# RKWin93/E2E-MAPPO-for-MT-FJSP

Measured on AMD Instinct MI355X. Metric: env-steps/sec (batched J6M6E2), higher is better.
Workload: dtype f64 (environment) / f32 (encoder: f32 storage and accumulation; 128x128 products on the 16-bit matrix cores from split f32 operands, f32-accurate: DESIGN.md §4)

## Files before the change

### __graft_entry__.py

```python
#!/usr/bin/env python3
import os
import sys

ROOT = os.path.dirname(os.path.abspath(__file__))
if ROOT not in sys.path:
    sys.path.insert(0, ROOT)


def build() -> None:
    from importlib import import_module
    import mtfjsp_amd
    _build = import_module("e2e-mappo-for-mt-fjsp_amd._build")
    lib = _build.build(force=True, verbose=True)
    capi = import_module("e2e-mappo-for-mt-fjsp_amd.capi")
    capi.lib()
    print("variant:", _build.build_variant("funcs", ["-DMTFJSP_BODY_FUNCS=3"]))
    from oracle import env_oracle
    print("oracle:", env_oracle.build(force=True))
    print("built", lib)


def smoke() -> None:
    import numpy as np
    import torch
    from importlib import import_module
    import mtfjsp_amd
    assert torch.cuda.is_available(), "smoke() needs cuda:0"
    batch_env = import_module("e2e-mappo-for-mt-fjsp_amd.batch_env")
    inst = import_module("e2e-mappo-for-mt-fjsp_amd.instances")
    from oracle.env_oracle import OracleBatch
    J, M, E, B = 6, 6, 2, 8
    T = J * M
    t, p, tt, edge = inst.generate_instances(B, J, M, E, seed=0)
    import random
    random.seed(0)
    w3 = inst.random_weights(B)
    env = batch_env.DeviceBatchEnv(J, M, E, B, obs_dtype="f64")
    env.load_instances(t, p, tt, edge=edge)
    env.scaler_init()
    env.reset(w3)
    orc = OracleBatch(t, p, tt, edge)
    orc.scaler_init()
    orc.reset(w3)
    a = torch.zeros(B, dtype=torch.int32, device=env.device); m = torch.zeros_like(a); j = torch.zeros_like(a)
    for s in range(T):
        env.random_actions(7, s, a, m, j)
        env.step(a, m)
        info, raw, _ = orc.step(a.cpu().numpy(), m.cpu().numpy())
        cand, mask = orc.job_mask_update(j.cpu().numpy())
        o = orc.observe()
        assert np.array_equal(env.info.cpu().numpy(), info), f"step {s}: rewards differ"
        assert np.array_equal(env.tasks_fea.cpu().numpy(), o["tfea"]), f"step {s}: tasks_fea differ"
        assert np.array_equal(env.dense_adj().cpu().numpy(), o["adj"]), f"step {s}: adj differ"
        assert np.array_equal(env.m_fea2.cpu().numpy(), o["mfea2"])
        assert np.array_equal(env.candidate.cpu().numpy(), cand) and np.array_equal(env.job_mask.cpu().numpy(), mask)
    assert bool(env.info[:, 1].all())
    _smoke_encoder()
    print("smoke OK: HIP env == oracle on", B, "instances x", T, "steps")


def _smoke_encoder() -> None:
    try:
        from importlib import import_module
        enc = import_module("e2e-mappo-for-mt-fjsp_amd.encoder")
    except ImportError:
        return
    if hasattr(enc, "smoke"):
        enc.smoke()


if __name__ == "__main__":
    cmd = sys.argv[1] if len(sys.argv) > 1 else "build"
    {"build": build, "smoke": smoke}[cmd]()
```

### e2e-mappo-for-mt-fjsp_amd/csrc/mtfjsp_gin_resident.h

```cpp
#pragma once
#include <type_traits>
#include <utility>

#ifndef GR_ABL
#define GR_ABL 0
#endif
#define GR_NT 18
#ifndef GR_NRES
#define GR_NRES 16
#endif
#ifndef GR_VRES
#define GR_VRES 1
#endif
#define GR_ROWS (32 * GR_NT)
#define GR_RING 6
#define GR_NBAR 6
#ifndef GR_GRP
#define GR_GRP 2
#endif
#ifndef GR_LOOK
#define GR_LOOK 2
#endif
#define GR_ROWB 272
#define GR_PLANE (32 * GR_ROWB)
#define GR_TILE (2 * GR_PLANE)
#define GR_MAXCAND 384
#define GR_MAXWARM 10
#define GR_MAXT 65
#define GR_MINT 16
#define GR_MAXIPC 64

#ifndef GR_MIX
#define GR_MIX 2
#endif
#ifndef GR_SETTLE
#define GR_SETTLE 1
#endif
#ifndef GR_FOLD_DPP
#define GR_FOLD_DPP 1
#endif
#ifndef GR_STAT_ASM
#define GR_STAT_ASM 0
#endif
#ifndef GR_PK
#define GR_PK 1
#endif
typedef float f32x16 __attribute__((ext_vector_type(16)));
typedef _Float16 gr_h8 __attribute__((ext_vector_type(8)));
typedef _Float16 gr_h2 __attribute__((ext_vector_type(2)));

struct GinResArgs {
    int B, T, J, ipc;
    const void *tfea; int feat_f64;
    const int *ell_col; const float *ell_val;
    const void *Wx32[6];
    float wsinv[6];
    const float *gamma[6], *beta[6];
    unsigned long long *stats;
    unsigned long long *stats_next;
    int wexp[6];
    int ffrac[6];
    unsigned long long *bar;
    unsigned long long epoch;
    unsigned *fail;
    unsigned *range_flag;
    const int *candidate;
    float *pooled;
    float *cand_feat;
    float *h_nodes;
    float *zspill;
    double inv_rows;
    int barrier_only;
    unsigned expect_extra;
    unsigned long long *stamps;
    const void *warm[GR_MAXWARM];
    unsigned warm_lines[GR_MAXWARM];
    int nwarm;
};
#define GR_STATS_PART (6 * 8 * HD * 2)
#define GR_STATS_SET GR_STATS_PART
#ifdef GR_STAMP
#define GR_STAMP_AT(i) do { if (tid == 0 && A.stamps) { A.stamps[(size_t)blockIdx.x * 64 + (i)] = __builtin_amdgcn_s_memrealtime(); \
                                                         if ((i) <= 30) A.stamps[(size_t)blockIdx.x * 64 + 33 + (i)] = __builtin_amdgcn_s_memtime(); } } while (0)
#else
#define GR_STAMP_AT(i) do { } while (0)
#endif

#define GR_OFF_PLANES 0
#define GR_OFF_RING (2 * GR_TILE)
#define GR_RING_BYTES ((2 * GR_LOOK - 2) * GR_TILE > GR_RING * 32 * HD * 4 ? (2 * GR_LOOK - 2) * GR_TILE : GR_RING * 32 * HD * 4)
#define GR_OFF_ELLC (GR_OFF_RING + GR_RING_BYTES)
#define GR_OFF_ELLV0 (GR_OFF_ELLC + GR_ROWS * 4)
#define GR_OFF_ELLV1 (GR_OFF_ELLV0 + GR_ROWS * 4)
#define GR_OFF_BN (GR_OFF_ELLV1 + GR_ROWS * 4)
#define GR_OFF_CAND (GR_OFF_BN + 2 * HD * 4)
#define GR_OFF_ZERO (GR_OFF_CAND + GR_ROWS * 4)
#define GR_OFF_FLAG (GR_OFF_ZERO + 2 * HD * 4)
#define GR_OFF_CNT (GR_OFF_FLAG + 64)
#define GR_LDS_BYTES (GR_OFF_CNT + 5 * (GR_NT / GR_GRP) * 4 + 12)
static size_t gin_res_lds_bytes() { return (size_t)GR_LDS_BYTES; }
static_assert(GR_LDS_BYTES <= 160 * 1024, "resident GIN kernel: LDS budget");

#if GR_PK == 1
__device__ __forceinline__ f32x2 gr_fma2(f32x2 a, f32x2 b, f32x2 c) { return __builtin_elementwise_fma(a, b, c); }
__device__ __forceinline__ f32x2 gr_add2(f32x2 a, f32x2 b) { return a + b; }
__device__ __forceinline__ f32x2 gr_sub2(f32x2 a, f32x2 b) { return a - b; }
__device__ __forceinline__ f32x2 gr_mul2(f32x2 a, f32x2 b) { return a * b; }
#else
#if GR_PK == 2
__device__ __forceinline__ float gr_pin(float x) { return x; }
#else
__device__ __forceinline__ float gr_pin(float x) { asm("" : "+v"(x)); return x; }
#endif
__device__ __forceinline__ f32x2 gr_fma2(f32x2 a, f32x2 b, f32x2 c) { return f32x2{gr_pin(__builtin_fmaf(a[0], b[0], c[0])), gr_pin(__builtin_fmaf(a[1], b[1], c[1]))}; }
__device__ __forceinline__ f32x2 gr_add2(f32x2 a, f32x2 b) { return f32x2{gr_pin(a[0] + b[0]), gr_pin(a[1] + b[1])}; }
__device__ __forceinline__ f32x2 gr_sub2(f32x2 a, f32x2 b) { return f32x2{gr_pin(a[0] - b[0]), gr_pin(a[1] - b[1])}; }
__device__ __forceinline__ f32x2 gr_mul2(f32x2 a, f32x2 b) { return f32x2{gr_pin(a[0] * b[0]), gr_pin(a[1] * b[1])}; }
#endif
__device__ __forceinline__ f32x2 gr_rem2(f32x2 v, gr_h2 p)
// ... 128 lines not shown
#pragma unroll
        for (int k = 0; k < NER; k++) {
            const int r = tid + 256 * k, rc = r < nrows ? r : nrows - 1;
            ecc[k] = *reinterpret_cast<const int2 *>(A.ell_col + (grow0 + rc) * 2);
            evv[k] = *reinterpret_cast<const float2 *>(A.ell_val + (grow0 + rc) * 2);
        }
#pragma unroll
        for (int k = 0; k < NF4; k++) reinterpret_cast<f32x4 *>(s_feat)[tid + 256 * k] = fpre[k];
        if (A.feat_f64) {
            const double *src = reinterpret_cast<const double *>(A.tfea) + grow0 * 12;
            const int n12 = nrows * 12;
            __syncthreads();
#pragma unroll 1
            for (int i0 = 0; i0 < n12; i0 += 256 * 9) {
                double d[9];
#pragma unroll
                for (int k = 0; k < 9; k++) { const int i = i0 + tid + 256 * k; d[k] = src[i < n12 ? i : n12 - 1]; }
#pragma unroll
                for (int k = 0; k < 9; k++) { const int i = i0 + tid + 256 * k; if (i < n12) s_feat[i] = (float)d[k]; }
            }
        }
#pragma unroll
        for (int k = 0; k < NER; k++) {
            const int r = tid + 256 * k;
            if (r < GR_ROWS) {
                unsigned cp = 0xffffffffu; float v0 = 0.f, v1 = 0.f;
                if (r < nrows) {
                    const int2 cc = ecc[k];
                    const float2 vv = evv[k];
                    const int base = (r / T) * T;
                    const unsigned r0 = cc.x >= 0 ? (unsigned)(base + cc.x) : 0xffffu, r1 = cc.y >= 0 ? (unsigned)(base + cc.y) : 0xffffu;
                    cp = r0 | (r1 << 16); v0 = cc.x >= 0 ? vv.x : 0.f; v1 = cc.y >= 0 ? vv.y : 0.f;
                }
                s_ellc[r] = cp; s_ellv0[r] = v0; s_ellv1[r] = v1; s_rowcand[r] = -1;
            }
        }
        {
            const f32x4 *wi = reinterpret_cast<const f32x4 *>(A.Wx32[0]) + (size_t)wave * (3 * 64) + lane;
            __builtin_amdgcn_sched_barrier(0);
#pragma unroll
            for (int p = 0; p < 3; p++) w0pre[p] = wi[p * 64];
            __builtin_amdgcn_sched_barrier(0);
        }
        if (tid == 0) s_flag[1] = 0u;
        if (tid < 5 * (GR_NT / GR_GRP)) s_cnt[tid] = 0u;
        for (int i = tid; i < 2 * GR_TILE / 16; i += 256) reinterpret_cast<float4 *>(s_planes)[i] = make_float4(0.f, 0.f, 0.f, 0.f);
        if (A.candidate) {
            LDS_BARRIER();
#pragma unroll
            for (int k = 0; k < (GR_MAXCAND + 255) / 256; k++) {
                const int i = tid + 256 * k, c = cand_pre[k];
                if (i < ninst * A.J && c >= 0 && c < T && atomicExch(&s_rowcand[(i / A.J) * T + c], i) != -1) s_flag[1] = 1u;
            }
        }
        s_zero[tid] = 0.f;
    }
    f32x16 acc[GR_NRES];
    f32x16 zs[2];
    float *zsp = A.zspill + ((size_t)(blockIdx.x * 4 + wave) * (GR_NT - GR_NRES)) * 1024 + lane * 4;
    auto zload = [&](auto Jc) __attribute__((always_inline)) {
        constexpr int j = decltype(Jc)::value;
        if constexpr (GR_VRES) return;
#pragma unroll
        for (int g = 0; g < 4; g++) {
            const float4 v = *reinterpret_cast<const float4 *>(zsp + j * 1024 + g * 256);
            zs[j & 1][4 * g] = v.x; zs[j & 1][4 * g + 1] = v.y; zs[j & 1][4 * g + 2] = v.z; zs[j & 1][4 * g + 3] = v.w;
        }
    };
    auto zstore = [&](auto Jc, const f32x16 &a) __attribute__((always_inline)) {
        constexpr int j = decltype(Jc)::value;
        if constexpr (GR_VRES) return;
#pragma unroll
        for (int g = 0; g < 4; g++) *reinterpret_cast<float4 *>(zsp + j * 1024 + g * 256) = make_float4(a[4 * g], a[4 * g + 1], a[4 * g + 2], a[4 * g + 3]);
    };
#define GR_TILEVAL(rt) ((rt) < GR_NRES ? acc[(rt) < GR_NRES ? (rt) : 0] : zs[(rt) >= GR_NRES ? ((rt) - GR_NRES) & 1 : 0])
    auto mfma_v = [&](f32x16 &c, const gr_h8 &a, const gr_h8 &b, bool zero) __attribute__((always_inline)) {
        if (zero) asm volatile("v_mfma_f32_32x32x16_f16 %0, %1, %2, 0" : "=v"(c) : "v"(a), "v"(b));
        else asm volatile("v_mfma_f32_32x32x16_f16 %0, %1, %2, %0" : "+v"(c) : "v"(a), "v"(b));
    };
    int nrows_l = nrows, n_l = n;
    bool timed_out = false;
    gr_h8 wf[2][8];
    bf16x8 w0f[3];
    f32x2 ts[8], tq[8];
#pragma unroll
    for (int i = 0; i < 8; i++) { ts[i] = f32x2{0.f, 0.f}; tq[i] = f32x2{0.f, 0.f}; }

    auto load_weights = [&](int layer) __attribute__((always_inline)) {
        const float4 *wi = reinterpret_cast<const float4 *>(A.Wx32[layer]) + (size_t)wave * (2 * 8 * 64) + lane;
#pragma unroll
        for (int p = 0; p < 2; p++)
#pragma unroll
            for (int ks = 0; ks < 8; ks++) wf[p][ks] = __builtin_bit_cast(gr_h8, wi[(p * 8 + ks) * 64]);
    };
    auto stat2 = [&](int i, float x, float y) __attribute__((always_inline)) {
        const f32x2 v = {x, y};
#if GR_STAT_ASM == 1
        asm volatile("v_pk_add_f32 %0, %2, %0\n\tv_pk_fma_f32 %1, %2, %2, %1" : "+v"(ts[i]), "+v"(tq[i]) : "v"(v));
#elif GR_STAT_ASM == 2
        float s0 = ts[i][0], s1 = ts[i][1], q0 = tq[i][0], q1 = tq[i][1];
        asm volatile("v_add_f32 %0, %4, %0\n\tv_add_f32 %1, %5, %1\n\tv_fma_f32 %2, %4, %4, %2\n\tv_fma_f32 %3, %5, %5, %3" : "+v"(s0), "+v"(s1), "+v"(q0), "+v"(q1) : "v"(x), "v"(y));
        ts[i] = f32x2{s0, s1}; tq[i] = f32x2{q0, q1};
#else
        ts[i] = gr_add2(ts[i], v); tq[i] = gr_fma2(v, v, tq[i]);
        asm volatile("" : "+v"(ts[i]), "+v"(tq[i]));
#endif
    };
    auto stats_all = [&](const f32x16 &a) __attribute__((always_inline)) {
        if (GR_ABL & 4) return;
#pragma unroll
        for (int i = 0; i < 8; i++) stat2(i, a[2 * i], a[2 * i + 1]);
    };
    auto split2x4 = [&](f32x2 v01, f32x2 v23, uint2 &p0, uint2 &p1) __attribute__((always_inline)) {
        const gr_h2 a = __builtin_convertvector(v01, gr_h2), b = __builtin_convertvector(v23, gr_h2);
#if GR_MIX == 2
        const gr_h2 c = gr_rem16(v01, a), d = gr_rem16(v23, b);
#else
        const f32x2 r01 = gr_rem2(v01, a), r23 = gr_rem2(v23, b);
        const gr_h2 c = __builtin_convertvector(r01, gr_h2), d = __builtin_convertvector(r23, gr_h2);
#endif
        p0 = make_uint2(__builtin_bit_cast(unsigned, a), __builtin_bit_cast(unsigned, b));
        p1 = make_uint2(__builtin_bit_cast(unsigned, c), __builtin_bit_cast(unsigned, d));
    };
    auto stats_tile = [&](auto Tc) __attribute__((always_inline)) {
        constexpr int RT = decltype(Tc)::value;
        stats_all(GR_TILEVAL(RT));
    };
    auto fold_stats = [&]() __attribute__((always_inline)) {
        float *red = s_ring;
        float *mine = red + (wave * 64 + lane) * 36;
#pragma unroll
        for (int j = 0; j < 4; j++) {
            *reinterpret_cast<float4 *>(mine + 4 * j) = make_float4(ts[2 * j][0], ts[2 * j][1], ts[2 * j + 1][0], ts[2 * j + 1][1]);
            *reinterpret_cast<float4 *>(mine + 16 + 4 * j) = make_float4(tq[2 * j][0], tq[2 * j][1], tq[2 * j + 1][0], tq[2 * j + 1][1]);
        }
#pragma unroll
        for (int i = 0; i < 8; i++) { ts[i] = f32x2{0.f, 0.f}; tq[i] = f32x2{0.f, 0.f}; }
        LDS_BARRIER();
        const int col = tid >> 1, kind = tid & 1, cw = col & 31;
        const float *src = red + ((col >> 5) * 64 + 32 * ((cw >> 2) & 1)) * 36 + 4 * (cw >> 3) + (cw & 3) + 16 * kind;
        float s0 = 0.f, s1 = 0.f, s2 = 0.f, s3 = 0.f;
#pragma unroll
        for (int i = 0; i < 32; i += 4) { s0 += src[i * 36]; s1 += src[(i + 1) * 36]; s2 += src[(i + 2) * 36]; s3 += src[(i + 3) * 36]; }
        return (s0 + s1) + (s2 + s3);
    };
    auto fold_stats_dpp = [&]() __attribute__((always_inline)) {
        const bool b4 = (lane & 16) != 0, b3 = (lane & 8) != 0, b2 = (lane & 4) != 0, b1 = (lane & 2) != 0, b0 = (lane & 1) != 0;
        auto dpp = [&](float x, auto Ctrl) __attribute__((always_inline)) {
            return __builtin_bit_cast(float, __builtin_amdgcn_update_dpp(0, __builtin_bit_cast(int, x), decltype(Ctrl)::value, 0xF, 0xF, true));
        };
        float v16[16];
#pragma unroll
        for (int c = 0; c < 16; c++) {
            const float a = ts[c >> 1][c & 1], q_ = tq[c >> 1][c & 1];
            v16[c] = (b4 ? q_ : a) + __shfl_xor(b4 ? a : q_, 16);
        }
#pragma unroll
        for (int i = 0; i < 8; i++) { ts[i] = f32x2{0.f, 0.f}; tq[i] = f32x2{0.f, 0.f}; }
        float v8[8];
#pragma unroll
        for (int c = 0; c < 8; c++) v8[c] = (b3 ? v16[c + 8] : v16[c]) + dpp(b3 ? v16[c] : v16[c + 8], std::integral_constant<int, 0x140>{});
        float v4[4];
#pragma unroll
        for (int c = 0; c < 4; c++) v4[c] = (b2 ? v8[c + 4] : v8[c]) + dpp(b2 ? v8[c] : v8[c + 4], std::integral_constant<int, 0x141>{});
        float v2[2];
#pragma unroll
// ... 13 lines not shown
        split2x4(f32x2{bn_relu_ss(a[4 * g], s4.x, h4.x), bn_relu_ss(a[4 * g + 1], s4.y, h4.y)},
                 f32x2{bn_relu_ss(a[4 * g + 2], s4.z, h4.z), bn_relu_ss(a[4 * g + 3], s4.w, h4.w)}, p0, p1);
        *reinterpret_cast<uint2 *>(dst) = p0;
        *reinterpret_cast<uint2 *>(dst + GR_PLANE) = p1;
    };
    auto produce_tile = [&](auto Tc, unsigned char *pbuf) __attribute__((always_inline)) {
        gr_static_for<4>([&](auto Gc) __attribute__((always_inline)) { produce_quarter(Tc, Gc, pbuf); });
        __builtin_amdgcn_sched_barrier(0);
    };
    const unsigned char *xa0 = s_planes + n * GR_ROWB + 16 * h;
#define GR_FENCE() __builtin_amdgcn_sched_barrier(0)
#define GR_PIN_V() do { } while (0)
    auto consume_tile = [&](auto Tc) __attribute__((always_inline)) {
        constexpr int RT = decltype(Tc)::value;
        constexpr int PT = RT + GR_LOOK;
        constexpr bool NEXT = (PT < GR_NT) && !(GR_ABL & 1);
        constexpr bool STATS = RT > 0 && (GR_VRES || RT - 1 < GR_NRES) && !(GR_ABL & 4);
        const unsigned char *xa = plane_buf(RT % (2 * GR_LOOK)) + n * GR_ROWB + 16 * h;
        unsigned char *pnext = plane_buf(PT % (2 * GR_LOOK));
        const float *bn = PT * 32 + n_l < nrows_l ? s_bn : s_zero;
        gr_h8 xf[2][2];
#pragma unroll
        for (int p = 0; p < 2; p++) xf[0][p] = *reinterpret_cast<const gr_h8 *>(xa + p * GR_PLANE);
        float4 s4 = make_float4(0.f, 0.f, 0.f, 0.f), h4 = s4;
        if constexpr (NEXT) {
            s4 = *reinterpret_cast<const float4 *>(bn + 32 * wave + 4 * h);
            h4 = *reinterpret_cast<const float4 *>(bn + HD + 32 * wave + 4 * h);
        }
        constexpr bool VT = GR_VRES && RT >= GR_NRES;
        f32x16 atmp;
        f32x16 &a = RT < GR_NRES ? acc[RT < GR_NRES ? RT : 0] : VT ? zs[RT >= GR_NRES ? (RT - GR_NRES) & 1 : 0] : atmp;
        if constexpr (RT + GR_LOOK + 1 >= GR_NRES && RT + GR_LOOK + 1 < GR_NT) zload(std::integral_constant<int, RT + GR_LOOK + 1 - GR_NRES>{});
        gr_static_for<4>([&](auto Pc) __attribute__((always_inline)) {
            constexpr int g = decltype(Pc)::value;
            const gr_h8 *x0 = xf[0], *x1 = xf[1];
            f32x2 v01 = {0.f, 0.f}, v23 = {0.f, 0.f}, e01 = v01, e23 = v01;
            gr_h2 p01 = {0, 0}, p23 = p01, q01 = p01, q23 = p01;
            unsigned char *dst = pnext + n * GR_ROWB + (32 * wave + 8 * g + 4 * h) * 2;
            const f32x16 &nx = GR_TILEVAL(PT < GR_NT ? PT : RT);
            const f32x16 &pv = GR_TILEVAL(RT > 0 ? RT - 1 : 0);
            auto M = [&](int ks, int wp, int xp) __attribute__((always_inline)) {
                if (GR_ABL & 2) return;
                if constexpr (VT) mfma_v(a, wf[wp][ks], (ks & 1) ? x1[xp] : x0[xp], ks == 0 && wp == 0 && xp == 1);
                else if (ks == 0 && wp == 0 && xp == 1)
                    a = __builtin_amdgcn_mfma_f32_32x32x16_f16(wf[wp][ks], x0[xp], f32x16{0.f, 0.f, 0.f, 0.f, 0.f, 0.f, 0.f, 0.f, 0.f, 0.f, 0.f, 0.f, 0.f, 0.f, 0.f, 0.f}, 0, 0, 0);
                else a = __builtin_amdgcn_mfma_f32_32x32x16_f16(wf[wp][ks], (ks & 1) ? x1[xp] : x0[xp], a, 0, 0, 0);
            };
            M(2 * g, 0, 1);
            xf[1][0] = *reinterpret_cast<const gr_h8 *>(xa + 32 * (2 * g + 1));
            if constexpr (NEXT) { v01 = gr_fma2(f32x2{nx[4 * g], nx[4 * g + 1]}, f32x2{s4.x, s4.y}, f32x2{h4.x, h4.y});
                                  v23 = gr_fma2(f32x2{nx[4 * g + 2], nx[4 * g + 3]}, f32x2{s4.z, s4.w}, f32x2{h4.z, h4.w}); }
            GR_FENCE();
            M(2 * g, 1, 0);
            xf[1][1] = *reinterpret_cast<const gr_h8 *>(xa + GR_PLANE + 32 * (2 * g + 1));
            if constexpr (NEXT) { v01 = __builtin_elementwise_max(v01, f32x2{0.f, 0.f}); v23 = __builtin_elementwise_max(v23, f32x2{0.f, 0.f}); }
            GR_FENCE();
            M(2 * g, 0, 0);
            if constexpr (NEXT) { p01 = __builtin_convertvector(v01, gr_h2); p23 = __builtin_convertvector(v23, gr_h2); }
            if constexpr (NEXT && g < 3) s4 = *reinterpret_cast<const float4 *>(bn + 32 * wave + 8 * (g + 1) + 4 * h);
            GR_FENCE();
            M(2 * g + 1, 0, 1);
            if constexpr (g < 3) xf[0][0] = *reinterpret_cast<const gr_h8 *>(xa + 32 * (2 * g + 2));
            if constexpr (NEXT && !GR_MIX) { e01 = __builtin_convertvector(p01, f32x2); e23 = __builtin_convertvector(p23, f32x2); }
            if constexpr (NEXT && g < 3) h4 = *reinterpret_cast<const float4 *>(bn + HD + 32 * wave + 8 * (g + 1) + 4 * h);
            GR_FENCE();
            M(2 * g + 1, 1, 0);
            if constexpr (g < 3) xf[0][1] = *reinterpret_cast<const gr_h8 *>(xa + GR_PLANE + 32 * (2 * g + 2));
            if constexpr (NEXT) { if constexpr (GR_MIX == 2) { q01 = gr_rem16(v01, p01); q23 = gr_rem16(v23, p23); }
                                  else if constexpr (GR_MIX == 1) { v01 = gr_rem2(v01, p01); v23 = gr_rem2(v23, p23); } else { v01 = gr_sub2(v01, e01); v23 = gr_sub2(v23, e23); }
                                  if (!(GR_ABL & 8)) *reinterpret_cast<uint2 *>(dst) = make_uint2(__builtin_bit_cast(unsigned, p01), __builtin_bit_cast(unsigned, p23));
                                  if constexpr (GR_MIX != 2) { q01 = __builtin_convertvector(v01, gr_h2); q23 = __builtin_convertvector(v23, gr_h2); } }
            GR_FENCE();
            M(2 * g + 1, 0, 0);
            if constexpr (NEXT) { if (!(GR_ABL & 8)) *reinterpret_cast<uint2 *>(dst + GR_PLANE) = make_uint2(__builtin_bit_cast(unsigned, q01), __builtin_bit_cast(unsigned, q23));
                                  else asm volatile("" :: "v"(p01), "v"(p23), "v"(q01), "v"(q23)); }
            if constexpr (STATS) { stat2(2 * g, pv[4 * g], pv[4 * g + 1]); stat2(2 * g + 1, pv[4 * g + 2], pv[4 * g + 3]); }
            GR_FENCE();
        });
        if constexpr (RT >= GR_NRES && !GR_VRES) {
            stats_all(a);
            zstore(std::integral_constant<int, RT - GR_NRES>{}, a);
            GR_FENCE();
        }
        if constexpr (!VT && GR_SETTLE) { asm volatile("s_nop 1"); GR_FENCE(); }
    };
    auto consume_tile0 = [&](auto Tc) __attribute__((always_inline)) {
        constexpr int RT = decltype(Tc)::value;
        const unsigned char *xa = xa0 + 32 * (RT & 7);
        bf16x8 x[3];
#pragma unroll
        for (int p = 0; p < 3; p++) x[p] = *reinterpret_cast<const bf16x8 *>(xa + p * GR_PLANE);
        f32x16 a = {0.f, 0.f, 0.f, 0.f, 0.f, 0.f, 0.f, 0.f, 0.f, 0.f, 0.f, 0.f, 0.f, 0.f, 0.f, 0.f};
        a = __builtin_amdgcn_mfma_f32_32x32x16_bf16(w0f[0], x[2], a, 0, 0, 0);
        a = __builtin_amdgcn_mfma_f32_32x32x16_bf16(w0f[2], x[0], a, 0, 0, 0);
        a = __builtin_amdgcn_mfma_f32_32x32x16_bf16(w0f[1], x[1], a, 0, 0, 0);
        a = __builtin_amdgcn_mfma_f32_32x32x16_bf16(w0f[0], x[1], a, 0, 0, 0);
        a = __builtin_amdgcn_mfma_f32_32x32x16_bf16(w0f[1], x[0], a, 0, 0, 0);
        a = __builtin_amdgcn_mfma_f32_32x32x16_bf16(w0f[0], x[0], a, 0, 0, 0);
        if constexpr (RT < GR_NRES) acc[RT] = a;
        else if constexpr (GR_VRES) zs[(RT - GR_NRES) & 1] = a;
        else {
            stats_all(a);
            zstore(std::integral_constant<int, RT - GR_NRES>{}, a);
        }
        if constexpr (RT > 0 && (GR_VRES || RT - 1 < GR_NRES)) stats_tile(std::integral_constant<int, RT - 1>{});
        __builtin_amdgcn_sched_barrier(0);
    };
    auto layer_boundary = [&](auto Kc) __attribute__((always_inline)) {
        constexpr int k = decltype(Kc)::value;
        GR_STAMP_AT(4 + 4 * k);
        if constexpr (GR_VRES && GR_NT > GR_NRES) {
            asm volatile("s_nop 15\n\ts_nop 15" ::: "memory");
            stats_all(zs[(GR_NT - 1 - GR_NRES) & 1]);
        }
#if GR_FOLD_DPP
        (void)fold_stats;
        const float colsum = fold_stats_dpp();
        const int kind = n >> 4, scol = 32 * wave + 8 * ((n & 15) >> 2) + 4 * h + (n & 3);
        constexpr int PAIR = 16;
#else
        const float colsum = fold_stats();
        const int kind = tid & 1, scol = tid >> 1;
        constexpr int PAIR = 1;
#endif
        const int sidx = 2 * scol + kind;
        if (k == 1) GR_STAMP_AT(2);
        const unsigned grp = blockIdx.x & 7u;
        {
            float x = colsum;
            if (!(__builtin_fabsf(x) * (kind ? A.wsinv[k] * A.wsinv[k] : A.wsinv[k]) < __builtin_ldexpf(1.0f, 51 - A.ffrac[k]))) {
                if (A.range_flag && !timed_out) __hip_atomic_store(A.range_flag, 1u, __ATOMIC_RELAXED, __HIP_MEMORY_SCOPE_SYSTEM);
                x = 0.f;
            }
            (void)__hip_atomic_fetch_add(A.stats + ((size_t)k * 8 + grp) * 256 + sidx, gr_fix_encode(x, kind ? 2 * A.wexp[k] : A.wexp[k], A.ffrac[k]),
                                         __ATOMIC_RELAXED, __HIP_MEMORY_SCOPE_AGENT);
        }
        if (k == 1) GR_STAMP_AT(3);
        const float ga = A.gamma[k][scol], be = A.beta[k][scol];
        if constexpr (k < 5) load_weights(k + 1);
        GR_STAMP_AT(5 + 4 * k);
        const unsigned long long *w0 = A.stats + (size_t)k * 8 * 256 + sidx;
        unsigned long long vw[8], want[8], ssum = 0;
#pragma unroll
        for (int j = 0; j < 8; j++) want[j] = (unsigned long long)((nblk >> 3) + ((unsigned)j < (nblk & 7u) ? 1u : 0u));
        {
            const unsigned long long t0 = __builtin_amdgcn_s_memrealtime();
            for (;;) {
#pragma unroll
                for (int j = 0; j < 8; j++) vw[j] = __hip_atomic_load(w0 + (size_t)j * 256, __ATOMIC_RELAXED, __HIP_MEMORY_SCOPE_AGENT);
                bool done = true;
                ssum = 0;
#pragma unroll
                for (int j = 0; j < 8; j++) { done = done && (vw[j] >> 58) == want[j]; ssum += vw[j] & GR_FIX_PAYLOAD; }
                if (__builtin_amdgcn_ballot_w64(!done) == 0ull) break;
                if (__builtin_amdgcn_s_memrealtime() - t0 > 400000ull) {
                    __hip_atomic_store(A.fail, 1u, __ATOMIC_RELAXED, __HIP_MEMORY_SCOPE_SYSTEM);
                    timed_out = true;
                    break;
                }
                __builtin_amdgcn_s_sleep(2);
            }
            GR_STAMP_AT(6 + 4 * k);
            const double tot = gr_fix_decode(ssum, nblk, A.ffrac[k]);
            const double oth = __shfl_xor(tot, PAIR);
            if (!kind) {
                const double mean = tot * A.inv_rows;
                double var = oth * A.inv_rows - mean * mean;
                if (var < 0) var = 0;
                const float rstd = 1.0f / sqrtf((float)(var + BN_EPS));
                const float s = rstd * ga;
                s_bn[scol] = s * A.wsinv[k];
                s_bn[HD + scol] = be - (float)mean * s;
            }
        }
        LDS_BARRIER();
        GR_STAMP_AT(7 + 4 * k);
    };

    GR_STAMP_AT(0);
#pragma unroll
    for (int p = 0; p < 3; p++) w0f[p] = __builtin_bit_cast(bf16x8, w0pre[p]);
    LDS_BARRIER();
    GR_STAMP_AT(1);
    {
        const float *s_feat = s_ring;
        auto produce0 = [&](int rt) __attribute__((always_inline)) {
            const int r = 8 * wave + (lane >> 3), fk = lane & 7, row = rt * 32 + r;
            const int fo = fk < 6 ? 2 * fk : 0;
            const unsigned cp = s_ellc[row];
            const unsigned r0 = cp & 0xffffu, r1 = cp >> 16;
            const int deg = 1 + (r0 != 0xffffu) + (r1 != 0xffffu);
            const float inv = deg == 1 ? 1.0f : deg == 2 ? 0.5f : (1.0f / 3.0f);
            const float w0 = s_ellv0[row], w1 = s_ellv1[row];
            const int n0 = r0 != 0xffffu ? (int)r0 : row, n1 = r1 != 0xffffu ? (int)r1 : row;
            const float2 o = *reinterpret_cast<const float2 *>(s_feat + row * 12 + fo);
            const float2 x = *reinterpret_cast<const float2 *>(s_feat + n0 * 12 + fo);
            const float2 y = *reinterpret_cast<const float2 *>(s_feat + n1 * 12 + fo);
            float v[4] = {__builtin_fmaf(w1, y.x, __builtin_fmaf(w0, x.x, o.x)) * inv, __builtin_fmaf(w1, y.y, __builtin_fmaf(w0, x.y, o.y)) * inv, 0.f, 0.f};
            if (row >= nrows) { v[0] = 0.f; v[1] = 0.f; }
            uint2 p0, p1, p2;
            split3x4(v, p0, p1, p2);
            unsigned char *d = s_planes + r * GR_ROWB + 32 * (rt & 7) + 4 * fk;
            if (fk < 6) {
                *reinterpret_cast<unsigned *>(d) = p0.x;
                *reinterpret_cast<unsigned *>(d + GR_PLANE) = p1.x;
                *reinterpret_cast<unsigned *>(d + 2 * GR_PLANE) = p2.x;
            }
        };
        gr_static_for<(GR_NT + 7) / 8>([&](auto Cc) __attribute__((always_inline)) {
            constexpr int C = decltype(Cc)::value;
            constexpr int NTC = GR_NT - 8 * C < 8 ? GR_NT - 8 * C : 8;
#pragma unroll
            for (int i = 0; i < NTC; i++) produce0(8 * C + i);
            LDS_BARRIER();
            __builtin_amdgcn_sched_barrier(0);
            gr_static_for<NTC>([&](auto Ic) __attribute__((always_inline)) {
                constexpr int RT = 8 * C + decltype(Ic)::value;
                consume_tile0(std::integral_constant<int, RT>{});
            });
            LDS_BARRIER();
            __builtin_amdgcn_sched_barrier(0);
        });
    }
    layer_boundary(std::integral_constant<int, 0>{});

    gr_static_for<5>([&](auto Lc) __attribute__((always_inline)) {
        constexpr int layer = decltype(Lc)::value + 1;
#ifndef GR_KEEP_MASKS
        asm volatile("" : "+s"(nrows_l), "+v"(n_l));
#endif
        if constexpr (layer != 3) {
            gr_static_for<GR_LOOK>([&](auto Ic) __attribute__((always_inline)) { produce_tile(Ic, plane_buf(decltype(Ic)::value)); });
            LDS_BARRIER();
            unsigned *cnt = s_cnt + (layer - 1) * (GR_NT / GR_GRP);
            gr_static_for<GR_NT>([&](auto Tc) __attribute__((always_inline)) {
                constexpr int RT = decltype(Tc)::value;
                constexpr int step = RT / GR_GRP, back = GR_LOOK / GR_GRP;
                if constexpr (GR_LOOK > GR_GRP && RT % GR_GRP == 0 && step >= back) {
                    while (__builtin_amdgcn_readfirstlane(__hip_atomic_load(&cnt[step - back], __ATOMIC_RELAXED, __HIP_MEMORY_SCOPE_WORKGROUP)) < 4u)
                        __builtin_amdgcn_s_sleep(1);
                    asm volatile("" ::: "memory");
                    __builtin_amdgcn_sched_barrier(0);
                }
                consume_tile(Tc);
                GR_PIN_V();
                if constexpr (RT % GR_GRP == GR_GRP - 1) {
                    if constexpr (GR_LOOK > GR_GRP) {
                        asm volatile("" ::: "memory");
                        if (lane == 0) __hip_atomic_fetch_add(&cnt[step], 1u, __ATOMIC_RELAXED, __HIP_MEMORY_SCOPE_WORKGROUP);
                    } else LDS_BARRIER();
                }
                __builtin_amdgcn_sched_barrier(0);
            });
            if constexpr (GR_LOOK > GR_GRP) LDS_BARRIER();
            static_assert(GR_NT % GR_GRP == 0 && GR_GRP >= 1 && (GR_LOOK == GR_GRP || GR_LOOK == 2 * GR_GRP) && GR_LOOK <= GR_NRES, "tile groups");
        } else {
            auto write_h = [&](auto Tc) __attribute__((always_inline)) {
                constexpr int rt = decltype(Tc)::value;
                float *base = s_ring + ((rt % GR_RING) * 32 + n) * HD;
                gr_static_for<4>([&](auto Gc) __attribute__((always_inline)) {
                    constexpr int g = decltype(Gc)::value;
                    const float *bn = rt * 32 + n_l < nrows_l ? s_bn : s_zero;
                    const float4 s4 = *reinterpret_cast<const float4 *>(bn + 32 * wave + 8 * g + 4 * h);
                    const float4 h4 = *reinterpret_cast<const float4 *>(bn + HD + 32 * wave + 8 * g + 4 * h);
                    const f32x16 &a = GR_TILEVAL(rt);
                    const int ch = (8 * wave + 2 * g + h) ^ (n & 7);
                    *reinterpret_cast<float4 *>(base + 4 * ch) = make_float4(bn_relu_ss(a[4 * g], s4.x, h4.x), bn_relu_ss(a[4 * g + 1], s4.y, h4.y),
                                                                             bn_relu_ss(a[4 * g + 2], s4.z, h4.z), bn_relu_ss(a[4 * g + 3], s4.w, h4.w));
                });
                __builtin_amdgcn_sched_barrier(0);
            };
            auto ring_row = [&](int R) __attribute__((always_inline)) {
                const int t = R >> 5;
                return ((t - GR_RING * ((t * 43) >> 8)) * 32 + (R & 31)) * HD;
            };
            struct AggRow { const float *po, *px, *py; float w0, w1, inv; int s0, s1, s2; };
            auto agg_row = [&](int RT) __attribute__((always_inline)) {
                AggRow r;
                const int row = RT * 32 + n_l;
                const unsigned cp = s_ellc[row];
                const unsigned r0 = cp & 0xffffu, r1 = cp >> 16;
                r.w0 = s_ellv0[row]; r.w1 = s_ellv1[row];
                const int deg = 1 + (r0 != 0xffffu) + (r1 != 0xffffu);
                r.inv = deg == 1 ? 1.0f : deg == 2 ? 0.5f : (1.0f / 3.0f);
                const int n0 = r0 != 0xffffu ? (int)r0 : row, n1 = r1 != 0xffffu ? (int)r1 : row;
                r.po = s_ring + ((RT % GR_RING) * 32 + n) * HD; r.px = s_ring + ring_row(n0); r.py = s_ring + ring_row(n1);
                r.s0 = n & 7; r.s1 = n0 & 7; r.s2 = n1 & 7;
                return r;
            };
            auto agg_quarter_standalone = [&](const AggRow &r, int g, unsigned char *dst) __attribute__((always_inline)) {
                const int chl = 8 * wave + 2 * g + h;
                const float4 o = *reinterpret_cast<const float4 *>(r.po + 4 * (chl ^ r.s0));
                const float4 x = *reinterpret_cast<const float4 *>(r.px + 4 * (chl ^ r.s1));
                const float4 y = *reinterpret_cast<const float4 *>(r.py + 4 * (chl ^ r.s2));
                const f32x2 W0 = {r.w0, r.w0}, W1 = {r.w1, r.w1}, IV = {r.inv, r.inv};
                const f32x2 v01 = gr_mul2(gr_fma2(W1, f32x2{y.x, y.y}, gr_fma2(W0, f32x2{x.x, x.y}, f32x2{o.x, o.y})), IV);
                const f32x2 v23 = gr_mul2(gr_fma2(W1, f32x2{y.z, y.w}, gr_fma2(W0, f32x2{x.z, x.w}, f32x2{o.z, o.w})), IV);
                uint2 p0, p1;
                split2x4(v01, v23, p0, p1);
                *reinterpret_cast<uint2 *>(dst + 16 * g) = p0;
                *reinterpret_cast<uint2 *>(dst + 16 * g + GR_PLANE) = p1;
            };
            auto consume_agg = [&](auto Tc) __attribute__((always_inline)) {
                constexpr int RT = decltype(Tc)::value;
                constexpr bool NEXT = RT + 1 < GR_NT && !(GR_ABL & 1);
                constexpr bool WH = RT + 4 < GR_NT && !(GR_ABL & 1);
                constexpr int WT = WH ? RT + 4 : RT;
                constexpr bool STATS = RT > 0 && (GR_VRES || RT - 1 < GR_NRES) && !(GR_ABL & 4);
                constexpr bool VT = GR_VRES && RT >= GR_NRES;
                const unsigned char *xa = xa0 + (RT & 1) * GR_TILE;
                gr_h8 xf[2][2];
#pragma unroll
                for (int p = 0; p < 2; p++) xf[0][p] = *reinterpret_cast<const gr_h8 *>(xa + p * GR_PLANE);
                AggRow r = agg_row(NEXT ? RT + 1 : RT);
// ... 121 lines not shown
#endif
#pragma unroll
        for (int rt = 0; rt < GR_NT; rt++) slot[rt] = (GR_ABL & 32) ? -1 : s_rowcand[rt * 32 + n_l];
        LDS_BARRIER();
        GR_STAMP_AT(28);
        float x[16];
        float4 w0, w1, w2, w3;
        auto pool_load = [&](int rt) __attribute__((always_inline)) {
            const float *rb = tb + (rt & 1) * (32 * 36) + (16 * h) * 36 + c;
#pragma unroll
            for (int i = 0; i < 16; i++) x[i] = rb[i * 36];
            const float4 *wt = reinterpret_cast<const float4 *>(s_wtab + (left < 16 ? left : 16) * 16);
            w0 = wt[0]; w1 = wt[1]; w2 = wt[2]; w3 = wt[3];
        };
        auto pool_math = [&](int rt) __attribute__((always_inline)) {
            f32x2 sa2 = gr_fma2(f32x2{x[0], x[1]}, f32x2{w0.x, w0.y}, f32x2{0.f, 0.f});
            sa2 = gr_fma2(f32x2{x[2], x[3]}, f32x2{w0.z, w0.w}, sa2);
            sa2 = gr_fma2(f32x2{x[4], x[5]}, f32x2{w1.x, w1.y}, sa2);
            sa2 = gr_fma2(f32x2{x[6], x[7]}, f32x2{w1.z, w1.w}, sa2);
            sa2 = gr_fma2(f32x2{x[8], x[9]}, f32x2{w2.x, w2.y}, sa2);
            sa2 = gr_fma2(f32x2{x[10], x[11]}, f32x2{w2.z, w2.w}, sa2);
            sa2 = gr_fma2(f32x2{x[12], x[13]}, f32x2{w3.x, w3.y}, sa2);
            sa2 = gr_fma2(f32x2{x[14], x[15]}, f32x2{w3.z, w3.w}, sa2);
            const f32x2 t2 = gr_add2(gr_add2(gr_add2(f32x2{x[0], x[1]}, f32x2{x[2], x[3]}), gr_add2(f32x2{x[4], x[5]}, f32x2{x[6], x[7]})),
                                     gr_add2(gr_add2(f32x2{x[8], x[9]}, f32x2{x[10], x[11]}), gr_add2(f32x2{x[12], x[13]}, f32x2{x[14], x[15]})));
            const float tot = t2[0] + t2[1];
            const float sa = sa2[0] + sa2[1];
            float *pp = s_part + ((2 * rt + h) * 2) * HD + 32 * wave + c;
            pp[0] = left >= 16 ? tot : sa; pp[HD] = left >= 16 ? 0.f : tot - sa;
            left -= 32;
            if (left <= 0) left += T;
            if (left <= 0) left += T;
        };
        gr_static_for<GR_NT>([&](auto Tc) __attribute__((always_inline)) {
            constexpr int rt = decltype(Tc)::value;
            const f32x16 &a = GR_TILEVAL(rt);
            if constexpr (rt > 0) { if (!(GR_ABL & 16)) pool_load(rt - 1); }
            float4 v[4];
#pragma unroll
            for (int g = 0; g < 4; g++) {
                const f32x2 lo = __builtin_elementwise_max(gr_fma2(f32x2{a[4 * g], a[4 * g + 1]}, f32x2{S[g].x, S[g].y}, f32x2{Hs[g].x, Hs[g].y}), f32x2{0.f, 0.f});
                const f32x2 hi = __builtin_elementwise_max(gr_fma2(f32x2{a[4 * g + 2], a[4 * g + 3]}, f32x2{S[g].z, S[g].w}, f32x2{Hs[g].z, Hs[g].w}), f32x2{0.f, 0.f});
                v[g] = make_float4(lo[0], lo[1], hi[0], hi[1]);
            }
            float *wb = tb + (rt & 1) * (32 * 36);
#pragma unroll
            for (int g = 0; g < 4; g++) *reinterpret_cast<float4 *>(wb + n * 36 + 8 * g + 4 * h) = v[g];
            if (slot[rt] >= 0) {
                float *d = A.cand_feat + ((size_t)inst0 * A.J + slot[rt]) * HD + 32 * wave + 4 * h;
#pragma unroll
                for (int g = 0; g < 4; g++) *reinterpret_cast<float4 *>(d + 8 * g) = v[g];
            }
            if (A.h_nodes && rt * 32 + n_l < nrows) {
                float *d = A.h_nodes + (grow0 + rt * 32 + n_l) * HD + 32 * wave + 4 * h;
#pragma unroll
                for (int g = 0; g < 4; g++) *reinterpret_cast<float4 *>(d + 8 * g) = v[g];
            }
            if constexpr (rt > 0) { if (!(GR_ABL & 16)) pool_math(rt - 1); }
            __builtin_amdgcn_sched_barrier(0);
        });
        if (!(GR_ABL & 16)) { pool_load(GR_NT - 1); pool_math(GR_NT - 1); }
        asm volatile("" :: "v"(warm_word));
        GR_STAMP_AT(29);
        LDS_BARRIER();
        const float invT = 1.0f / (float)T;
        static_assert(GR_MAXT <= 65, "an instance spans at most five 16-row chunks");
        for (int item = tid; item < ninst * HD; item += 256) {
            const int inst = item >> 7, col = item & (HD - 1);
            const int r0 = inst * T, k0 = r0 >> 4, k1 = (r0 + T - 1) >> 4;
            float pv[5];
#pragma unroll
            for (int kk = 0; kk < 5; kk++) {
                const int k = k0 + kk < k1 ? k0 + kk : k1;
                pv[kk] = s_part[(2 * k + (16 * k < r0 ? 1 : 0)) * HD + col];
            }
            float sum = 0.f;
#pragma unroll
            for (int kk = 0; kk < 5; kk++) sum = k0 + kk <= k1 ? sum + pv[kk] : sum;
            A.pooled[(size_t)inst0 * HD + item] = sum * invT;
        }
        if (A.candidate && s_flag[1]) {
            __threadfence();
            __syncthreads();
            for (int i = wave; i < ninst * A.J; i += 4) {
                const int cnd = A.candidate[(size_t)inst0 * A.J + i];
                if (cnd < 0 || cnd >= T) continue;
                const int win = s_rowcand[(i / A.J) * T + cnd];
                if (win != i) {
                    const float2 x = *reinterpret_cast<const float2 *>(A.cand_feat + ((size_t)inst0 * A.J + win) * HD + 2 * lane);
                    *reinterpret_cast<float2 *>(A.cand_feat + ((size_t)inst0 * A.J + i) * HD + 2 * lane) = x;
                }
            }
        }
    }
    GR_STAMP_AT(31);
}
#endif
```

Measured before the change: 20.62 million.

## Add cross-tile software-pipelined GIN consume loop with register-carried operands

Adds a new consume path for the GIN encoder layers. It carries the next tile's X fragments and batch-norm scale/shift in registers across tile boundaries, interleaves their LDS loads with the MFMAs, and issues the per-pair LDS counter increment and spin-wait in inline assembly in the middle of the last MFMA group. The point is to hide LDS load latency and the inter-wave barrier cost at tile boundaries. In exchange it raises register pressure and adds hand-written exec-mask asm, and it changes a lane index in the candidate-feature copy.

Result: no change. 20.68 million (median of 2 runs) (+0.3%).

```diff
diff --git a/__graft_entry__.py b/__graft_entry__.py
--- a/__graft_entry__.py
+++ b/__graft_entry__.py
@@ -15,6 +15,7 @@
     capi = import_module("e2e-mappo-for-mt-fjsp_amd.capi")
     capi.lib()
     print("variant:", _build.build_variant("funcs", ["-DMTFJSP_BODY_FUNCS=3"]))
+    print("variant:", _build.build_variant("xtile0", ["-DGR_XTILE=0"]))
     from oracle import env_oracle
     print("oracle:", env_oracle.build(force=True))
     print("built", lib)
diff --git a/e2e-mappo-for-mt-fjsp_amd/csrc/mtfjsp_gin_resident.h b/e2e-mappo-for-mt-fjsp_amd/csrc/mtfjsp_gin_resident.h
--- a/e2e-mappo-for-mt-fjsp_amd/csrc/mtfjsp_gin_resident.h
+++ b/e2e-mappo-for-mt-fjsp_amd/csrc/mtfjsp_gin_resident.h
@@ -35,6 +35,12 @@
 #endif
 #ifndef GR_SETTLE
 #define GR_SETTLE 1
+#endif
+#ifndef GR_XTILE
+#define GR_XTILE 1
+#endif
+#ifndef GR_XHAND
+#define GR_XHAND 1
 #endif
 #ifndef GR_FOLD_DPP
 #define GR_FOLD_DPP 1
@@ -329,6 +335,8 @@
     bool timed_out = false;
     gr_h8 wf[2][8];
     bf16x8 w0f[3];
+    gr_h8 xfc[2];
+    float4 s4c = make_float4(0.f, 0.f, 0.f, 0.f), h4c = s4c;
     f32x2 ts[8], tq[8];
 #pragma unroll
     for (int i = 0; i < 8; i++) { ts[i] = f32x2{0.f, 0.f}; tq[i] = f32x2{0.f, 0.f}; }
@@ -508,6 +516,93 @@
             zstore(std::integral_constant<int, RT - GR_NRES>{}, a);
             GR_FENCE();
         }
+        if constexpr (!VT && GR_SETTLE) { asm volatile("s_nop 1"); GR_FENCE(); }
+    };
+    typedef __attribute__((address_space(3))) unsigned char gr_lds_u8;
+    auto consume_tile_x = [&](auto Tc, unsigned *cnt) __attribute__((always_inline)) {
+        constexpr int RT = decltype(Tc)::value;
+        constexpr bool XB = GR_XHAND != 0, ODD = (RT & 1) != 0, LAST = RT + 1 >= GR_NT;
+        constexpr int PT = RT + 2, PT3 = RT + 3;
+        constexpr bool STATS = RT > 0 && !(GR_ABL & 4);
+        constexpr bool CARRY = !LAST && (XB || !ODD);
+        static_assert(GR_VRES, "GR_XTILE: the tiles beyond GR_NRES live in vector registers");
+        const unsigned char *xa = plane_buf(RT % 4) + n * GR_ROWB + 16 * h;
+        const unsigned char *xn = plane_buf((RT + 1) % 4) + n * GR_ROWB + 16 * h;
+        const unsigned cnt_addr = (unsigned)(size_t)(gr_lds_u8 *)smem + (unsigned)((const unsigned char *)(cnt + RT / 2) - smem);
+        gr_h8 xf1[2];
+        if constexpr (RT == 0) {
+#pragma unroll
+            for (int p = 0; p < 2; p++) xfc[p] = *reinterpret_cast<const gr_h8 *>(xa + p * GR_PLANE);
+            if constexpr (!(GR_ABL & 1)) {
+                const float *bn2 = PT * 32 + n_l < nrows_l ? s_bn : s_zero;
+                s4c = *reinterpret_cast<const float4 *>(bn2 + 32 * wave + 8 * (XB ? 1 : 0) + 4 * h);
+                h4c = *reinterpret_cast<const float4 *>(bn2 + HD + 32 * wave + 8 * (XB ? 1 : 0) + 4 * h);
+            }
+        }
+        constexpr bool VT = RT >= GR_NRES;
+        f32x16 &a = RT < GR_NRES ? acc[RT < GR_NRES ? RT : 0] : zs[RT >= GR_NRES ? (RT - GR_NRES) & 1 : 0];
+        gr_static_for<4>([&](auto Pc) __attribute__((always_inline)) {
+            constexpr int g = decltype(Pc)::value;
+            constexpr int q = g + (XB ? 1 : 0), qn = q + 1;
+            constexpr int QT = q < 4 ? PT : PT3, QQ = q & 3, NQT = qn < 4 ? PT : PT3, NQQ = qn & 3;
+            constexpr bool NEXT = QT < GR_NT && !(GR_ABL & 1), PRE = NQT < GR_NT && !(GR_ABL & 1);
+            const float *bnn = NQT * 32 + n_l < nrows_l ? s_bn : s_zero;
+            const gr_h8 *x0 = xfc, *x1 = xf1;
+            f32x2 v01 = {0.f, 0.f}, v23 = {0.f, 0.f}, e01 = v01, e23 = v01;
+            gr_h2 p01 = {0, 0}, p23 = p01, q01 = p01, q23 = p01;
+            unsigned char *dst = plane_buf(QT % 4) + n * GR_ROWB + (32 * wave + 8 * QQ + 4 * h) * 2;
+            const f32x16 &nx = GR_TILEVAL(QT < GR_NT ? QT : RT);
+            const f32x16 &pv = GR_TILEVAL(RT > 0 ? RT - 1 : 0);
+            auto M = [&](int ks, int wp, int xp) __attribute__((always_inline)) {
+                if (GR_ABL & 2) return;
+                if constexpr (VT) mfma_v(a, wf[wp][ks], (ks & 1) ? x1[xp] : x0[xp], ks == 0 && wp == 0 && xp == 1);
+                else if (ks == 0 && wp == 0 && xp == 1)
+                    a = __builtin_amdgcn_mfma_f32_32x32x16_f16(wf[wp][ks], x0[xp], f32x16{0.f, 0.f, 0.f, 0.f, 0.f, 0.f, 0.f, 0.f, 0.f, 0.f, 0.f, 0.f, 0.f, 0.f, 0.f, 0.f}, 0, 0, 0);
+                else a = __builtin_amdgcn_mfma_f32_32x32x16_f16(wf[wp][ks], (ks & 1) ? x1[xp] : x0[xp], a, 0, 0, 0);
+            };
+            M(2 * g, 0, 1);
+            xf1[0] = *reinterpret_cast<const gr_h8 *>(xa + 32 * (2 * g + 1));
+            if constexpr (NEXT) { v01 = gr_fma2(f32x2{nx[4 * QQ], nx[4 * QQ + 1]}, f32x2{s4c.x, s4c.y}, f32x2{h4c.x, h4c.y});
+                                  v23 = gr_fma2(f32x2{nx[4 * QQ + 2], nx[4 * QQ + 3]}, f32x2{s4c.z, s4c.w}, f32x2{h4c.z, h4c.w}); }
+            GR_FENCE();
+            M(2 * g, 1, 0);
+            xf1[1] = *reinterpret_cast<const gr_h8 *>(xa + GR_PLANE + 32 * (2 * g + 1));
+            if constexpr (NEXT) { v01 = __builtin_elementwise_max(v01, f32x2{0.f, 0.f}); v23 = __builtin_elementwise_max(v23, f32x2{0.f, 0.f}); }
+            GR_FENCE();
+            M(2 * g, 0, 0);
+            if constexpr (NEXT) { p01 = __builtin_convertvector(v01, gr_h2); p23 = __builtin_convertvector(v23, gr_h2); }
+            if constexpr (PRE) s4c = *reinterpret_cast<const float4 *>(bnn + 32 * wave + 8 * NQQ + 4 * h);
+            if constexpr (XB && ODD && !LAST && g == 3) {
+                unsigned long long ex; unsigned av;
+                asm volatile("s_mov_b64 %0, exec\n\ts_mov_b64 exec, 1\n\tv_mov_b32 %1, %2\n\tds_inc_u32 %1, %1\n\ts_mov_b64 exec, %0" : "=&s"(ex), "=&v"(av) : "s"(cnt_addr) : "memory");
+            }
+            GR_FENCE();
+            M(2 * g + 1, 0, 1);
+            if constexpr (XB && ODD && !LAST && g == 3) {
+                unsigned seen_v, seen_s;
+                asm volatile(".Lgr_wait_%=:\n\tv_mov_b32 %0, %2\n\tds_read_b32 %0, %0\n\ts_waitcnt lgkmcnt(0)\n\tv_readfirstlane_b32 %1, %0\n\ts_cmp_ge_u32 %1, 4\n\t"
+                             "s_cbranch_scc1 .Lgr_go_%=\n\ts_sleep 1\n\ts_branch .Lgr_wait_%=\n.Lgr_go_%=:"
+                             : "=&v"(seen_v), "=&s"(seen_s) : "s"(cnt_addr) : "memory", "scc");
+            }
+            if constexpr (g < 3) xfc[0] = *reinterpret_cast<const gr_h8 *>(xa + 32 * (2 * g + 2));
+            else if constexpr (CARRY) xfc[1] = *reinterpret_cast<const gr_h8 *>(xn + GR_PLANE);
+            if constexpr (NEXT && !GR_MIX) { e01 = __builtin_convertvector(p01, f32x2); e23 = __builtin_convertvector(p23, f32x2); }
+            if constexpr (PRE) h4c = *reinterpret_cast<const float4 *>(bnn + HD + 32 * wave + 8 * NQQ + 4 * h);
+            GR_FENCE();
+            M(2 * g + 1, 1, 0);
+            if constexpr (g < 3) xfc[1] = *reinterpret_cast<const gr_h8 *>(xa + GR_PLANE + 32 * (2 * g + 2));
+            else if constexpr (CARRY) xfc[0] = *reinterpret_cast<const gr_h8 *>(xn);
+            if constexpr (NEXT) { if constexpr (GR_MIX == 2) { q01 = gr_rem16(v01, p01); q23 = gr_rem16(v23, p23); }
+                                  else if constexpr (GR_MIX == 1) { v01 = gr_rem2(v01, p01); v23 = gr_rem2(v23, p23); } else { v01 = gr_sub2(v01, e01); v23 = gr_sub2(v23, e23); }
+                                  if (!(GR_ABL & 8)) *reinterpret_cast<uint2 *>(dst) = make_uint2(__builtin_bit_cast(unsigned, p01), __builtin_bit_cast(unsigned, p23));
+                                  if constexpr (GR_MIX != 2) { q01 = __builtin_convertvector(v01, gr_h2); q23 = __builtin_convertvector(v23, gr_h2); } }
+            GR_FENCE();
+            M(2 * g + 1, 0, 0);
+            if constexpr (NEXT) { if (!(GR_ABL & 8)) *reinterpret_cast<uint2 *>(dst + GR_PLANE) = make_uint2(__builtin_bit_cast(unsigned, q01), __builtin_bit_cast(unsigned, q23));
+                                  else asm volatile("" :: "v"(p01), "v"(p23), "v"(q01), "v"(q23)); }
+            if constexpr (STATS) { stat2(2 * g, pv[4 * g], pv[4 * g + 1]); stat2(2 * g + 1, pv[4 * g + 2], pv[4 * g + 3]); }
+            GR_FENCE();
+        });
         if constexpr (!VT && GR_SETTLE) { asm volatile("s_nop 1"); GR_FENCE(); }
     };
     auto consume_tile0 = [&](auto Tc) __attribute__((always_inline)) {
@@ -655,7 +750,29 @@
 #ifndef GR_KEEP_MASKS
         asm volatile("" : "+s"(nrows_l), "+v"(n_l));
 #endif
-        if constexpr (layer != 3) {
+        if constexpr (layer != 3 && GR_XTILE) {
+            static_assert(!GR_XTILE || (GR_LOOK == 2 && GR_GRP == 2), "GR_XTILE: four plane buffers, tiles in pairs");
+            produce_tile(std::integral_constant<int, 0>{}, plane_buf(0));
+            produce_tile(std::integral_constant<int, 1>{}, plane_buf(1));
+            if constexpr (GR_XHAND && !(GR_ABL & 1)) {
+                produce_quarter(std::integral_constant<int, 2>{}, std::integral_constant<int, 0>{}, plane_buf(2));
+                __builtin_amdgcn_sched_barrier(0);
+            }
+            LDS_BARRIER();
+            unsigned *cnt = s_cnt + (layer - 1) * (GR_NT / GR_GRP);
+            gr_static_for<GR_NT>([&](auto Tc) __attribute__((always_inline)) {
+                constexpr int RT = decltype(Tc)::value;
+                consume_tile_x(Tc, cnt);
+                if constexpr (RT % 2 == 1 && (!GR_XHAND || RT == GR_NT - 1)) {
+                    LDS_BARRIER();
+                    if constexpr (RT + 1 < GR_NT) {
+#pragma unroll
+                        for (int p = 0; p < 2; p++) xfc[p] = *reinterpret_cast<const gr_h8 *>(plane_buf((RT + 1) % 4) + n * GR_ROWB + 16 * h + p * GR_PLANE);
+                    }
+                }
+                __builtin_amdgcn_sched_barrier(0);
+            });
+        } else if constexpr (layer != 3) {
             gr_static_for<GR_LOOK>([&](auto Ic) __attribute__((always_inline)) { produce_tile(Ic, plane_buf(decltype(Ic)::value)); });
             LDS_BARRIER();
             unsigned *cnt = s_cnt + (layer - 1) * (GR_NT / GR_GRP);
@@ -943,13 +1060,14 @@
         if (A.candidate && s_flag[1]) {
             __threadfence();
             __syncthreads();
+            const int lane_t = GR_XTILE ? n_l + 32 * h : lane;
             for (int i = wave; i < ninst * A.J; i += 4) {
                 const int cnd = A.candidate[(size_t)inst0 * A.J + i];
                 if (cnd < 0 || cnd >= T) continue;
                 const int win = s_rowcand[(i / A.J) * T + cnd];
                 if (win != i) {
-                    const float2 x = *reinterpret_cast<const float2 *>(A.cand_feat + ((size_t)inst0 * A.J + win) * HD + 2 * lane);
-                    *reinterpret_cast<float2 *>(A.cand_feat + ((size_t)inst0 * A.J + i) * HD + 2 * lane) = x;
+                    const float2 x = *reinterpret_cast<const float2 *>(A.cand_feat + ((size_t)inst0 * A.J + win) * HD + 2 * lane_t);
+                    *reinterpret_cast<float2 *>(A.cand_feat + ((size_t)inst0 * A.J + i) * HD + 2 * lane_t) = x;
                 }
             }
         }
```
